# NyanCAD/Cadnip.jl

Hardware: AMD Instinct MI355X
Metric: newton_iters_per_sec (higher is better)
Workload: dtype f64; 1 GPU; gf180 DFF transient 0-700 ns (synthetic sp_mos1 level-1 card, 30 MOSFETs, n=235, nnz=1090), 4096 Vdd x temp corner instances per GPU (state resident in HBM; one 8-instance workgroup per CU in flight, the rest handed out by the kernel's instance queue); step = DC init + full transient of the batch; instances_per_gpu=4096, instances_total=4096, fused=2, newton_mode=1, launches_last_step=5120, accepted_last_step=6078488, rejected_last_step=692364

## Files before the change

### cadnip.jl_amd/csrc/api.hip

```cpp
#include <hip/hip_runtime.h>
#include <functional>
#include <algorithm>
#include <initializer_list>
#include <stdio.h>
#include <string.h>
#include <string>
#include <vector>
#include "internal.hpp"
#include "lu_transpose.hpp"
#include "va_generated.hpp"

using namespace cadnip;

namespace {
template <class T>
int dev_alloc(T** p, size_t count) {
  if (count == 0) count = 1;
  HIP_TRY(hipMalloc((void**)p, count * sizeof(T)));
  HIP_TRY(hipMemset(*p, 0, count * sizeof(T)));
  return CADNIP_OK;
}
template <class T>
int dev_upload(T** p, const T* src, size_t count) {
  int rc = dev_alloc(p, count);
// ... 949 lines not shown
int cadnip_sync(CadnipHandle* h) { if (!h) return CADNIP_BADARG; HIP_TRY(hipStreamSynchronize(h->stream)); return CADNIP_OK; }

int cadnip_profile_enable(CadnipHandle* h, int32_t on) {
  if (!h) return CADNIP_BADARG;
  h->prof_on = on != 0;
  h->prof.clear();
  return CADNIP_OK;
}
int cadnip_profile_read(CadnipHandle* h, int32_t max_entries, const char** names, double* ms, int64_t* calls) {
  if (!h) return 0;
  int k = 0;
  for (auto& e : h->prof) { if (k >= max_entries) break; names[k] = e.name; ms[k] = e.ms; calls[k] = e.calls; ++k; }
  return k;
}

}

namespace cadnip {
int restore_masks(CadnipHandle* h, bool cold) {
  const std::vector<int> ones((size_t)h->B, 1);
  if (cold) HIP_TRY(hipMemcpy(h->d_cold, ones.data(), ones.size() * sizeof(int), hipMemcpyHostToDevice));
  HIP_TRY(hipMemcpy(h->d_active, ones.data(), ones.size() * sizeof(int), hipMemcpyHostToDevice));
  return CADNIP_OK;
}

int upload_homotopy(CadnipHandle* h, const double* gshunt, const double* srcfact) {
  ++h->graph_epoch;
  const size_t B = (size_t)h->B;
  std::vector<double> g(B, h->spec.gshunt), sf(B, h->spec.srcFact);
  if (gshunt) g.assign(gshunt, gshunt + B);
  if (srcfact) sf.assign(srcfact, srcfact + B);
  bool any = false;
  for (size_t i = 0; i < B; ++i) if (g[i] != 0.0 || sf[i] < 1.0) any = true;
  HIP_TRY(hipMemcpy(h->d_gshunt, g.data(), B * sizeof(double), hipMemcpyHostToDevice));
  HIP_TRY(hipMemcpy(h->d_srcfact, sf.data(), B * sizeof(double), hipMemcpyHostToDevice));
  HIP_TRY(hipStreamSynchronize(h->stream));
  h->homotopy = any;
  return CADNIP_OK;
}
int upload_lu(CadnipHandle* h) {
  ++h->graph_epoch;
  LUProgram& P = h->lu;
  int** olds[] = {&h->d_load_src, &h->d_load_dst, &h->d_ent_pos, &h->d_ent_diag, &h->d_ent_ptr, &h->d_term_a, &h->d_term_b, &h->d_lev_ptr,
                  &h->d_lu_rowptr, &h->d_lu_col, &h->d_lu_diag, &h->d_rperm, &h->d_cperm, &h->d_fwd_rows, &h->d_fwd_lev_ptr, &h->d_bwd_rows, &h->d_bwd_lev_ptr};
  for (int** p : olds) if (*p) { (void)hipFree(*p); *p = nullptr; }
  if (h->d_LU) { (void)hipFree(h->d_LU); h->d_LU = nullptr; }
  std::vector<int> dst(h->nnz, 0);
  for (size_t k = 0; k < P.load_src.size(); ++k) dst[P.load_src[k]] = P.load_dst[k];
  TRY(dev_upload(&h->d_load_dst, dst));
  TRY(dev_upload(&h->d_ent_pos, P.ent_pos)); TRY(dev_upload(&h->d_ent_diag, P.ent_diag)); TRY(dev_upload(&h->d_ent_ptr, P.ent_ptr));
  TRY(dev_upload(&h->d_term_a, P.term_a)); TRY(dev_upload(&h->d_term_b, P.term_b)); TRY(dev_upload(&h->d_lev_ptr, P.lev_ptr));
  TRY(dev_upload(&h->d_lu_rowptr, P.lu_rowptr)); TRY(dev_upload(&h->d_lu_col, P.lu_col)); TRY(dev_upload(&h->d_lu_diag, P.lu_diag));
  TRY(dev_upload(&h->d_rperm, P.rperm)); TRY(dev_upload(&h->d_cperm, P.cperm));
  TRY(dev_upload(&h->d_fwd_rows, P.fwd_rows)); TRY(dev_upload(&h->d_fwd_lev_ptr, P.fwd_lev_ptr));
  TRY(dev_upload(&h->d_bwd_rows, P.bwd_rows)); TRY(dev_upload(&h->d_bwd_lev_ptr, P.bwd_lev_ptr));
  TRY(dev_alloc(&h->d_LU, (size_t)h->B * P.nnz_lu));
  h->analyzed = true;
  h->f2.dirty = true;
  h->ac.dirty = true;
  return CADNIP_OK;
}
}
```

### cadnip.jl_amd/csrc/dc_chain.hpp

```cpp
#pragma once
#include <algorithm>
#include <cmath>
#include <cstddef>
#include <vector>

namespace cadnip {

struct DCLogEntry { int inst, stage; double value; int ok; long long iters; };

struct DCChainOpts {
  int use_pcnr, cold_start, fused, use_stepping;
  bool has_limits;
  double gshunt, srcFact;
  const int* participate;
};

struct DCRun {
  int stage, use_pcnr, cold_start, fused;
  const int* part;
  const double* u;
  const double *gshunt, *srcFact;
  int* status;
  long long* iters;
  double *R, *R_direct;
  int B;
  double* dest() const {
    if (!R_direct) return R;
    for (int i = 0; i < B; ++i) if (status[i] != 1) return R;
    return R_direct;
  }
};

struct DCChainResult {
  long long iters = 0;
  int n_failed = 0;
  bool direct = false;
// ... 24 lines not shown
      s.factor = std::sqrt(s.factor);
    }
    return s.steps >= 20 ? GAVE_UP : AGAIN;
  }
};

struct SourceRule {
  struct State { double src = 0.0, conv = 0.0, raise = 0.1; int steps = 0; };
  double value(const State& s) const { return s.src; }
  Next digest(State& s, bool ok) const {
    ++s.steps;
    if (ok) {
      s.conv = s.src;
      if (s.src >= 1.0) return SOLVED;
      s.src = std::fmin(s.src + s.raise, 1.0);
    } else {
      if (s.src - s.conv < 1e-6) return GAVE_UP;
      s.raise /= 2.0;
      s.src = s.conv + s.raise;
    }
    return s.steps >= 50 ? GAVE_UP : AGAIN;
  }
};

template <class Rule> struct Ladder { typename Rule::State s; bool over = false; std::vector<double> u; };

}

template <class Runner>
int dc_chain(const DCChainOpts& o, int B_, int n_, double* u, int* converged, Runner&& runner, std::vector<DCLogEntry>& log, DCChainResult& res) {
  using namespace dc_chain_detail;
  const size_t B = (size_t)B_, n = (size_t)n_;
  res = DCChainResult();
  std::vector<double> start, U, R(B * n);
  std::vector<int> fin(B, 0), status(B), part(B, 1);
  std::vector<long long> iters(B);
  std::vector<double> gsh(B, o.gshunt), sfc(B, o.srcFact);
  auto masked = [&](size_t i) { return o.participate && !o.participate[i]; };
  for (size_t i = 0; i < B; ++i) if (masked(i)) { part[i] = 0; fin[i] = 1; }
  auto n_open = [&]() { int k = 0; for (size_t i = 0; i < B; ++i) k += !fin[i]; return k; };
  auto row = [&](std::vector<double>& v, size_t i) { return v.begin() + i * n; };
  auto run = [&](int stage, int use_pcnr, int cold_start, int fused, const double* from, const double* rung, double* R_direct) -> int {
    const DCRun r{stage, use_pcnr, cold_start, fused, part.data(), from, gsh.data(), sfc.data(), status.data(), iters.data(), R.data(), R_direct, B_};
    if (int rc = runner(r)) return rc;
    res.direct = R_direct && r.dest() == R_direct;
    for (size_t i = 0; i < B; ++i)
      if (part[i]) { res.iters += iters[i]; log.push_back({(int)i, stage, rung ? rung[i] : 0.0, status[i] == 1 ? 1 : 0, iters[i]}); }
    return 0;
  };
  auto take_all = [&]() { for (size_t i = 0; i < B; ++i) if (part[i]) { std::copy(row(R, i), row(R, i + 1), row(U, i)); if (status[i] == 1) fin[i] = 1; } };
  auto stepping = [&](int stage, auto rule, std::vector<double>& term, double spec_value) -> int {
    std::vector<Ladder<decltype(rule)>> L(B);
    for (size_t i = 0; i < B; ++i) { L[i].over = fin[i]; if (!fin[i]) L[i].u.assign(n, 0.0); }
    for (;;) {
      int k = 0;
      for (size_t i = 0; i < B; ++i) {
        part[i] = !L[i].over;
        term[i] = part[i] ? rule.value(L[i].s) : spec_value;
        if (part[i]) { ++k; std::copy(L[i].u.begin(), L[i].u.end(), row(U, i)); }
      }
      if (!k) return 0;
      if (int rc = run(stage, 0, 0, 0, U.data(), term.data(), nullptr)) return rc;
      for (size_t i = 0; i < B; ++i) {
        if (!part[i]) continue;
        const bool ok = status[i] == 1;
        if (ok) L[i].u.assign(row(R, i), row(R, i + 1));
        const Next next = rule.digest(L[i].s, ok);
        if (next == AGAIN) continue;
        L[i].over = true;
        fin[i] = next == SOLVED;
        std::copy(L[i].u.begin(), L[i].u.end(), row(U, i));
      }
    }
  };
  if (n_open())
    if (int rc = run(0, o.use_pcnr, o.cold_start, o.fused, u, nullptr, o.participate ? nullptr : u)) return rc;
  if (res.direct) {
    if (converged) std::fill(converged, converged + B, 1);
    return 0;
  }
  start.assign(u, u + B * n);
  U = start;
  take_all();
  if (n_open() && o.use_pcnr && o.has_limits) {
    for (size_t i = 0; i < B; ++i) { part[i] = !fin[i]; if (part[i]) std::copy(row(start, i), row(start, i + 1), row(U, i)); }
    if (int rc = run(1, 0, 0, 0, U.data(), nullptr, nullptr)) return rc;
    take_all();
  }
  if (n_open() && o.use_stepping)
    if (int rc = stepping(2, GshuntRule(o.gshunt), gsh, o.gshunt)) return rc;
  if (n_open() && o.use_stepping)
    if (int rc = stepping(3, SourceRule(), sfc, o.srcFact)) return rc;
  res.n_failed = n_open();
  std::copy(U.begin(), U.end(), u);
  if (converged) for (size_t i = 0; i < B; ++i) converged[i] = masked(i) ? 0 : fin[i];
  return 0;
}

}
```

### cadnip.jl_amd/csrc/driver.hip

```cpp
#include <hip/hip_runtime.h>
#include <chrono>
#include <string.h>
#include <vector>
#include "internal.hpp"
#include "dc_chain.hpp"

using namespace cadnip;

struct Driver {
  int n_save = 0, n_obs = 0, n_break = 0;
  double *t = nullptr, *h = nullptr, *hprev = nullptr, *hpp = nullptr;
  int *nhist = nullptr, *order = nullptr, *k = nullptr, *status = nullptr, *bp_idx = nullptr, *save_idx = nullptr, *dcstate = nullptr, *action = nullptr;
  long long* cnt = nullptr;
  double *mn_a0f = nullptr, *mn_ss = nullptr, *mn_dnp = nullptr; int* mn_flags = nullptr;
  double *u0 = nullptr, *u1 = nullptr, *u2 = nullptr, *up = nullptr, *beta = nullptr;
  double *u3 = nullptr, *hp3 = nullptr;
  double *atol = nullptr, *emask = nullptr, *breaks = nullptr, *save_t = nullptr, *out = nullptr;
  int* obs = nullptr;
  int* nactive = nullptr;
  int* part = nullptr;
  size_t out_cap = 0, brk_cap = 0, save_cap = 0, obs_cap = 0;
  std::vector<DCLogEntry> dc_log;
};

namespace {
#define TRY(x) do { int _rc = (x); if (_rc) return _rc; } while (0)
template <class T> int dalloc(T** p, size_t c) { if (*p) return CADNIP_OK; HIP_TRY(hipMalloc((void**)p, (c ? c : 1) * sizeof(T))); HIP_TRY(hipMemset(*p, 0, (c ? c : 1) * sizeof(T))); return CADNIP_OK; }
template <class T> int drealloc(T** p, size_t* cap, size_t c) { if (*p && *cap >= c) return CADNIP_OK; if (*p) (void)hipFree(*p); *p = nullptr; *cap = c; return dalloc(p, c); }

template <class F> int each_buffer(Driver* d, size_t B, size_t n, F f) {
  const size_t later = 0;
  TRY(f(&d->t, B)); TRY(f(&d->h, B)); TRY(f(&d->hprev, B)); TRY(f(&d->hpp, B));
  TRY(f(&d->nhist, B)); TRY(f(&d->order, B)); TRY(f(&d->k, B)); TRY(f(&d->status, B));
  TRY(f(&d->bp_idx, B)); TRY(f(&d->save_idx, B)); TRY(f(&d->dcstate, B)); TRY(f(&d->action, B));
  TRY(f(&d->cnt, B * 4));
  TRY(f(&d->mn_a0f, B)); TRY(f(&d->mn_ss, B)); TRY(f(&d->mn_dnp, B)); TRY(f(&d->mn_flags, B));
  TRY(f(&d->u0, B * n)); TRY(f(&d->u1, B * n)); TRY(f(&d->u2, B * n)); TRY(f(&d->up, B * n)); TRY(f(&d->beta, B * n));
  TRY(f(&d->atol, n)); TRY(f(&d->emask, n)); TRY(f(&d->nactive, 2)); TRY(f(&d->part, B));
  TRY(f(&d->u3, later)); TRY(f(&d->hp3, later));
  TRY(f(&d->breaks, later)); TRY(f(&d->save_t, later)); TRY(f(&d->obs, later)); TRY(f(&d->out, later));
  return CADNIP_OK;
}

int ensure_driver(CadnipHandle* h) {
  if (!h->drv) h->drv = new Driver();
  return each_buffer(h->drv, h->B, h->n, [](auto** p, size_t c) { return c ? dalloc(p, c) : CADNIP_OK; });
}

}
#include "tran_ctrl.hpp"
namespace {
__global__ void __launch_bounds__(64) k_tran_init(TranArgs a) {
  const int inst = blockIdx.x, tid = threadIdx.x, n = a.n;
  double* u = a.u + (size_t)inst * n;
  double* u0 = a.u0 + (size_t)inst * n;
  for (int i = tid; i < n; i += 64) { double v = u[i]; u0[i] = v; a.u1[(size_t)inst * n + i] = v; a.u2[(size_t)inst * n + i] = v; }
  int bp = 0;
  while (bp < a.n_break && a.breaks[bp] <= a.t0) ++bp;
  int si = 0;
  while (si < a.n_save && a.save_t[si] <= a.t0) {
    double* o = a.out + ((size_t)inst * a.n_save + si) * a.n_obs;
// ... 205 lines not shown
      for (int i = 0; i < h->B && victim < 0; ++i) if (stat[i] == -2) victim = i;
      if (victim >= 0) {
        ++repivots;
        std::vector<int> act((size_t)h->B);
        for (int i = 0; i < h->B; ++i) act[i] = (stat[i] == 0 || stat[i] == -2) ? 1 : 0;
        HIP_TRY(hipMemcpy(h->d_active, act.data(), act.size() * sizeof(int), hipMemcpyHostToDevice));
        rc = launch_jacobian(h); if (rc) break;
        HIP_TRY(hipStreamSynchronize(h->stream));
        if (cadnip_analyze(h, victim) == CADNIP_OK) {
          for (int i = 0; i < h->B; ++i) if (stat[i] == -2) stat[i] = 0;
          HIP_TRY(hipMemcpy(d->status, stat.data(), stat.size() * sizeof(int), hipMemcpyHostToDevice));
          rc = count_running(h, &running); if (rc) break;
        } else {
          for (int i = 0; i < h->B; ++i) act[i] = stat[i] == 0 ? 1 : 0;
          HIP_TRY(hipMemcpy(h->d_active, act.data(), act.size() * sizeof(int), hipMemcpyHostToDevice));
        }
      }
    }
    prev_running = running;
    if (running == 0) break;
  }
  h->initjct = saved_initjct;
  return rc;
}

}

extern "C" {

void cadnip_driver_free(CadnipHandle* h) {
  if (!h || !h->drv) return;
  Driver* d = h->drv;
  (void)each_buffer(d, 0, 0, [](auto** p, size_t) { if (*p) (void)hipFree(*p); return CADNIP_OK; });
  delete d;
  h->drv = nullptr;
}

int cadnip_tran_state(CadnipHandle* h, double* t_host, double* h_host, int32_t* order_host) {
  if (!h || !h->drv) return CADNIP_NOTREADY;
  Driver* d = h->drv;
  size_t B = h->B;
  if (t_host) HIP_TRY(hipMemcpy(t_host, d->t, B * sizeof(double), hipMemcpyDeviceToHost));
  if (h_host) HIP_TRY(hipMemcpy(h_host, d->h, B * sizeof(double), hipMemcpyDeviceToHost));
  if (order_host) HIP_TRY(hipMemcpy(order_host, d->order, B * sizeof(int), hipMemcpyDeviceToHost));
  return CADNIP_OK;
}

int cadnip_dc_run(CadnipHandle* h, const CadnipDCOpts* o, double* u_host, int32_t* converged_host, CadnipRunStats* st) {
  if (!h || !o || !u_host) return CADNIP_BADARG;
  TRY(ensure_driver(h));
  Driver* d = h->drv;
  const size_t B = h->B, n = h->n;
  auto w0 = std::chrono::steady_clock::now();
  d->dc_log.clear();
  if (!h->analyzed) {
    HIP_TRY(hipMemcpy(h->d_u, u_host, B * n * sizeof(double), hipMemcpyHostToDevice));
    TRY(restore_masks(h, false));
    TRY_RC(dev_zero_async(h, h->d_gamma, B * sizeof(double)));
    TRY_RC(dev_zero_async(h, h->d_t, B * sizeof(double)));
    std::vector<double> g(B, 1e9);
    int ij = h->initjct;
    h->initjct = (o->cold_start && o->use_pcnr && h->n_limits > 0) ? 1 : 0;
    int rc = launch_rebuild(h);
    h->initjct = ij;
    if (rc) return rc;
    HIP_TRY(hipMemcpy(h->d_gamma, g.data(), B * sizeof(double), hipMemcpyHostToDevice));
    TRY(launch_jacobian(h));
    HIP_TRY(hipStreamSynchronize(h->stream));
    TRY(cadnip_analyze(h, 0));
  }
  struct HomotopyGuard {
    CadnipHandle* h;
    ~HomotopyGuard() { (void)upload_homotopy(h, nullptr, nullptr); }
  } guard{h};
  std::vector<long long> cnt(B * 4);
  auto device_run = [&](const DCRun& r) -> int {
    HIP_TRY(hipMemcpy(h->d_u, r.u, B * n * sizeof(double), hipMemcpyHostToDevice));
    HIP_TRY(hipMemcpy(d->part, r.part, B * sizeof(int), hipMemcpyHostToDevice));
    TRY(upload_homotopy(h, r.gshunt, r.srcFact));
    TRY(dc_newton(h, o->abstol, o->maxiters, r.use_pcnr, r.cold_start, r.fused, d->part));
    HIP_TRY(hipMemcpy(r.status, d->status, B * sizeof(int), hipMemcpyDeviceToHost));
    HIP_TRY(hipMemcpy(r.dest(), h->d_u, B * n * sizeof(double), hipMemcpyDeviceToHost));
    HIP_TRY(hipMemcpy(cnt.data(), d->cnt, B * 4 * sizeof(long long), hipMemcpyDeviceToHost));
    for (size_t i = 0; i < B; ++i) r.iters[i] = cnt[i * 4];
    return CADNIP_OK;
  };
  const DCChainOpts chain{o->use_pcnr, o->cold_start, o->fused, o->use_stepping, h->n_limits > 0, h->spec.gshunt, h->spec.srcFact, o->participate};
  DCChainResult res;
  TRY(dc_chain(chain, h->B, h->n, u_host, converged_host, device_run, d->dc_log, res));
  if (!res.direct) HIP_TRY(hipMemcpy(h->d_u, u_host, B * n * sizeof(double), hipMemcpyHostToDevice));
  TRY(restore_masks(h, true));
  if (st) {
    memset(st, 0, sizeof(*st));
    st->newton_iters = res.iters;
    st->n_failed = res.n_failed;
    st->wall_seconds = std::chrono::duration<double>(std::chrono::steady_clock::now() - w0).count();
  }
  return res.n_failed ? CADNIP_NOCONV : CADNIP_OK;
}

int32_t cadnip_dc_log_size(CadnipHandle* h) { return (h && h->drv) ? (int32_t)h->drv->dc_log.size() : 0; }
int cadnip_dc_log_get(CadnipHandle* h, int32_t* inst, int32_t* stage, double* value, int32_t* ok, int64_t* iters) {
  if (!h || !h->drv) return CADNIP_NOTREADY;
  size_t k = 0;
  for (auto& e : h->drv->dc_log) {
    if (inst) inst[k] = e.inst; if (stage) stage[k] = e.stage; if (value) value[k] = e.value; if (ok) ok[k] = e.ok; if (iters) iters[k] = e.iters;
    ++k;
  }
  return CADNIP_OK;
}

int cadnip_tran_run(CadnipHandle* h, const CadnipTranOpts* o, double* out_host, int64_t* per_inst_host, CadnipRunStats* st) {
  if (!h || !o || !o->abstol || o->t1 <= o->t0 || o->n_save < 0 || o->n_break < 0) return CADNIP_BADARG;
  if (!h->analyzed) return CADNIP_NOTREADY;
  for (int i = 1; i < o->n_break; ++i) if (!(o->breaks[i] > o->breaks[i - 1])) return CADNIP_BADARG;
  for (int i = 1; i < o->n_save; ++i) if (!(o->save_t[i] >= o->save_t[i - 1])) return CADNIP_BADARG;
  for (int i = 0; i < o->n_obs; ++i) if (o->obs[i] < 0 || o->obs[i] >= h->n) return CADNIP_BADARG;
  TRY(ensure_driver(h));
  Driver* d = h->drv;
  const size_t B = h->B, n = h->n;
  const int n_obs = o->n_obs > 0 ? o->n_obs : (int)n;
  TRY(drealloc(&d->breaks, &d->brk_cap, (size_t)o->n_break));
  TRY(drealloc(&d->save_t, &d->save_cap, (size_t)o->n_save));
  TRY(drealloc(&d->obs, &d->obs_cap, (size_t)n_obs));
  TRY(drealloc(&d->out, &d->out_cap, B * (size_t)o->n_save * n_obs));
  if (o->n_break) HIP_TRY(hipMemcpy(d->breaks, o->breaks, o->n_break * sizeof(double), hipMemcpyHostToDevice));
  if (o->n_save) HIP_TRY(hipMemcpy(d->save_t, o->save_t, o->n_save * sizeof(double), hipMemcpyHostToDevice));
  std::vector<int> obs(n_obs);
  for (int i = 0; i < n_obs; ++i) obs[i] = o->n_obs > 0 ? o->obs[i] : i;
  HIP_TRY(hipMemcpy(d->obs, obs.data(), n_obs * sizeof(int), hipMemcpyHostToDevice));
  HIP_TRY(hipMemcpy(d->atol, o->abstol, n * sizeof(double), hipMemcpyHostToDevice));
  std::vector<double> emask(n, 1.0);
  int n_err = (int)n;
  if (o->err_mask) { n_err = 0; for (size_t i = 0; i < n; ++i) { emask[i] = o->err_mask[i] != 0.0 ? 1.0 : 0.0; n_err += emask[i] != 0.0; } }
  HIP_TRY(hipMemcpy(d->emask, emask.data(), n * sizeof(double), hipMemcpyHostToDevice));
  HIP_TRY(hipStreamSynchronize(h->stream));
  if (o->max_order >= 3) { TRY(dalloc(&d->u3, B * n)); TRY(dalloc(&d->hp3, B)); }
  TranArgs a = tran_args(h, o, n_obs, n_err);
  const bool delayed = h->dly.n_term > 0;
  if (delayed) { a.hmax = fmin(a.hmax, h->dly.tau_min); a.h0 = fmin(a.h0, a.hmax); }
  struct DelayGuard { CadnipHandle* h; bool on; ~DelayGuard() { if (on) { (void)launch_delay_clear(h); (void)hipStreamSynchronize(h->stream); } } } delay_guard{h, delayed};
  const bool use_fused = o->fused && fused2_plan(h, F2_TRAN, o->newton_mode).circuit_ok;
  struct ModeGuard { CadnipHandle* h; int saved; ~ModeGuard() { h->spec.mode = saved; } } mode_guard{h, h->spec.mode};
  h->spec.mode = 1;
  hipLaunchKernelGGL(k_tran_init, dim3(h->B), dim3(64), 0, h->stream, a);
  if (delayed) TRY(launch_delay_init(h, a.t0));
  HIP_TRY(hipStreamSynchronize(h->stream));
  auto w0 = std::chrono::steady_clock::now();
  int64_t launches = 0;
  const int64_t max_it = o->max_iterations > 0 ? o->max_iterations : 50000000;
  int rc = CADNIP_OK, running = h->B;
  const int check_every = use_fused ? 1024 : 8;
  if (use_fused) {
    hipEvent_t ev[2] = {nullptr, nullptr};
    HIP_TRY(hipEventCreateWithFlags(&ev[0], hipEventDisableTiming));
    HIP_TRY(hipEventCreateWithFlags(&ev[1], hipEventDisableTiming));
    int slot = 0;
    bool have_prev = false;
    while (launches < max_it) {
      rc = launch_fused2_rounds(h, a, check_every); if (rc) break;
      launches += check_every;
      rc = enqueue_running_count(h, slot); if (rc) break;
      if (hipEventRecord(ev[slot], h->stream) != hipSuccess) { rc = CADNIP_HIPERROR; break; }
      if (have_prev) {
        if (hipEventSynchronize(ev[1 - slot]) != hipSuccess) { rc = CADNIP_HIPERROR; break; }
        running = ((volatile int*)h->h_pinned)[1 - slot];
        if (running == 0) break;
      }
      have_prev = true;
      slot ^= 1;
    }
    hipError_t es = hipStreamSynchronize(h->stream);
    (void)hipEventDestroy(ev[0]); (void)hipEventDestroy(ev[1]);
    if (es != hipSuccess) { set_last_error("hipStreamSynchronize", es); return CADNIP_HIPERROR; }
    if (!rc && running > 0) rc = count_running(h, &running);
  }
  while (!use_fused && running > 0 && launches < max_it) {
    for (int c = 0; c < check_every; ++c) {
      rc = launch_rebuild(h); if (rc) break;
      if (delayed) { rc = launch_delay_apply(h, d->status); if (rc) break; }
      rc = launch_residual(h, h->d_du); if (rc) break;
      rc = launch_factor_solve(h, true, h->d_resid, h->d_delta); if (rc) break;
      { ProfScope ps(h, "tran_update");
        if (h->n >= 4096) hipLaunchKernelGGL(k_tran_update<256>, dim3(h->B), dim3(256), 0, h->stream, a);
        else hipLaunchKernelGGL(k_tran_update<64>, dim3(h->B), dim3(64), 0, h->stream, a); }
      if (delayed) { rc = launch_delay_record(h, d->t, d->u0, d->status); if (rc) break; }
      ++launches;
    }
    if (rc) break;
    rc = count_running(h, &running); if (rc) break;
  }
  HIP_TRY(hipStreamSynchronize(h->stream));
  double wall = std::chrono::duration<double>(std::chrono::steady_clock::now() - w0).count();
  if (rc) return rc;
  std::vector<long long> cnt(B * 4);
  std::vector<int> status(B);
  HIP_TRY(hipMemcpy(cnt.data(), d->cnt, B * 4 * sizeof(long long), hipMemcpyDeviceToHost));
  HIP_TRY(hipMemcpy(status.data(), d->status, B * sizeof(int), hipMemcpyDeviceToHost));
  if (out_host && o->n_save) HIP_TRY(hipMemcpy(out_host, d->out, B * (size_t)o->n_save * n_obs * sizeof(double), hipMemcpyDeviceToHost));
  CadnipRunStats s; memset(&s, 0, sizeof(s));
  for (size_t i = 0; i < B; ++i) {
    s.newton_iters += cnt[i * 4 + 0]; s.steps_accepted += cnt[i * 4 + 1]; s.steps_rejected += cnt[i * 4 + 2]; s.newton_failures += cnt[i * 4 + 3];
    if (status[i] != 1) s.n_failed += 1;
    if (per_inst_host) { per_inst_host[i * 4 + 0] = cnt[i * 4 + 0]; per_inst_host[i * 4 + 1] = cnt[i * 4 + 1]; per_inst_host[i * 4 + 2] = cnt[i * 4 + 2]; per_inst_host[i * 4 + 3] = status[i]; }
  }
  s.launches = launches; s.wall_seconds = wall;
  if (st) *st = s;
  TRY(restore_masks(h, false));
  return s.n_failed ? CADNIP_NOCONV : CADNIP_OK;
}

}
```

### cadnip.jl_amd/csrc/internal.hpp

```cpp
#pragma once
#include <hip/hip_runtime.h>
#include <stdint.h>
#include <string>
#include <vector>
#include "../../include/cadnip_hip.h"
#include "stamp_plan.hpp"
#include "ac_hbm_plan.hpp"
#include "delay_plan.hpp"
#define CADNIP_MOS1_PAR_OXCAP 8
#define CADNIP_MOS1_PAR_GD 30
#define CADNIP_MOS1_PAR_GS 31

#define HIP_TRY(expr)                                                     \
  do {                                                                    \
    hipError_t _e = (expr);                                               \
    if (_e != hipSuccess) {                                               \
      cadnip::set_last_error(#expr, _e);                                  \
      return CADNIP_HIPERROR;                                             \
    }                                                                     \
  } while (0)

namespace cadnip {

void set_last_error(const char* what, hipError_t e);
// ... 130 lines not shown
  template <class F> void each_buffer(F f) {
    f((void**)&d_pos); f((void**)&d_taps); f((void**)&d_rows); f((void**)&d_row_ptr); f((void**)&d_term_tap); f((void**)&d_row_store);
    f((void**)&d_tau); f((void**)&d_w); f((void**)&d_W); f((void**)&d_hist_t); f((void**)&d_hist_v); f((void**)&d_v_init);
    f((void**)&d_head); f((void**)&d_count);
  }
};

}

struct CadnipHandle {
  int device = 0;
  hipStream_t stream = nullptr;
  int B = 0;
  int n = 0, n_nodes = 0, n_currents = 0, n_charges = 0, n_limits = 0, nnz = 0;
  std::vector<int> h_rowptr, h_colidx, h_to_ref;
  std::vector<int> h_g_ptr, h_g_slots, h_c_ptr, h_c_slots, h_b_ptr, h_b_slots;
  int ns_g = 0, ns_c = 0, ns_b = 0, ns = 0;
  std::vector<cadnip::DeviceBlock> blocks;
  std::vector<double> h_limit_init;
  CadnipSpec spec{1, 1e-12, 0.0, 1.0};
  int initjct = 0;
  int *d_rowptr = nullptr, *d_colidx = nullptr, *d_to_ref = nullptr;
  int *d_g_ptr = nullptr, *d_g_slots = nullptr, *d_c_ptr = nullptr, *d_c_slots = nullptr, *d_b_ptr = nullptr, *d_b_slots = nullptr;
  unsigned char* d_diag_flag = nullptr;
  int* d_long_rows = nullptr;
  int n_long_rows = 0;
  double* d_dump = nullptr;
  unsigned* d_prep = nullptr;
  int n_prep = 0, n_prep_atomic = 0;
  bool prep_stale = true;
  double* d_wave = nullptr;
  double* d_limit_init = nullptr;
  double *d_gshunt = nullptr, *d_srcfact = nullptr;
  bool homotopy = false;
  double *d_u = nullptr, *d_du = nullptr, *d_t = nullptr, *d_gamma = nullptr;
  double *d_G = nullptr, *d_C = nullptr, *d_b = nullptr, *d_J = nullptr, *d_resid = nullptr, *d_delta = nullptr;
  double *d_limit_w = nullptr, *d_LU = nullptr, *d_tmp = nullptr;
  int* d_flags = nullptr;
  int* d_active = nullptr;
  int* d_nonfinite = nullptr;
  int* d_cold = nullptr;
  bool analyzed = false;
  cadnip::LUProgram lu;
  int *d_load_src = nullptr, *d_load_dst = nullptr, *d_ent_pos = nullptr, *d_ent_diag = nullptr, *d_ent_ptr = nullptr;
  int *d_term_a = nullptr, *d_term_b = nullptr, *d_lev_ptr = nullptr;
  int *d_lu_rowptr = nullptr, *d_lu_col = nullptr, *d_lu_diag = nullptr, *d_rperm = nullptr, *d_cperm = nullptr;
  int *d_fwd_rows = nullptr, *d_fwd_lev_ptr = nullptr, *d_bwd_rows = nullptr, *d_bwd_lev_ptr = nullptr;
  std::vector<unsigned char> leaf_unit_ok;
  cadnip::LULeaves leaves;
  bool va_ext = false;
  cadnip::FusedState f2;
  cadnip::AcState ac;
  cadnip::DelayState dly;
  struct Driver* drv = nullptr;
  bool prof_on = false;
  std::vector<cadnip::ProfEntry> prof;
  hipEvent_t ev0 = nullptr, ev1 = nullptr;
  int* h_pinned = nullptr;
  int* d_pinned = nullptr;
  char* h_stage = nullptr; char* d_stage = nullptr; size_t stage_bytes = 0, stage_off = 0;
  struct PendingDown { void* dst; const void* src; size_t bytes; };
  struct StepGraph { hipGraphExec_t exec = nullptr; unsigned long long epoch = 0, warmed = 0; };
  StepGraph step_graph[4];
  unsigned long long graph_epoch = 1;
  std::vector<PendingDown> stage_pending;
};
// ... 76 lines not shown
```

### cadnip.jl_amd/hip.py

```python
import ctypes as C
import os

import numpy as np

from .structure import Structure, TYPE_ID, type_id

_HERE = os.path.dirname(os.path.abspath(__file__))
LIB_PATH = os.environ.get("CADNIP_HIP_LIB") or os.path.join(_HERE, "libcadnip_hip.so")

OK, BADARG, SINGULAR, NONFINITE, HIPERROR, NOTREADY, NOCONV = range(7)
STATUS_NAMES = {0: "CADNIP_OK", 1: "CADNIP_BADARG", 2: "CADNIP_SINGULAR", 3: "CADNIP_NONFINITE",
                4: "CADNIP_HIPERROR", 5: "CADNIP_NOTREADY", 6: "CADNIP_NOCONV"}

AC_BREAKDOWN_TOL = 6e-9
AC_MEMORY = {"lds": 0, "hbm": 1, "auto": 2}

EXPORTS = [
    "cadnip_create", "cadnip_destroy", "cadnip_set_params", "cadnip_set_spec", "cadnip_set_initjct",
    "cadnip_rebuild", "cadnip_residual", "cadnip_jacobian", "cadnip_jacobian_dense", "cadnip_ode_rhs", "cadnip_ode_jacobian", "cadnip_get_GCb", "cadnip_get_contributions", "cadnip_analyze",
    "cadnip_analyze_values", "cadnip_factor", "cadnip_solve", "cadnip_factor_solve", "cadnip_lu_order", "cadnip_ac_solve", "cadnip_ac_adjoint", "cadnip_ac_solve_multi", "cadnip_ac_adjoint_multi", "cadnip_ac_sens", "cadnip_ac_arnoldi", "cadnip_ac_set_memory", "cadnip_ac_set_overlay", "cadnip_ac_plan_info", "cadnip_newton_step", "cadnip_newton_step_fused", "cadnip_debug_step_time", "cadnip_lu_stats", "cadnip_dc_run",
    "cadnip_dc_log_size", "cadnip_dc_log_get", "cadnip_tran_set_delay", "cadnip_tran_delay_info", "cadnip_tran_run", "cadnip_tran_state", "cadnip_dev_ptr", "cadnip_stream", "cadnip_set_u", "cadnip_get_u", "cadnip_get_flags",
    "cadnip_sync", "cadnip_debug_copy", "cadnip_debug_stamp_time", "cadnip_profile_enable", "cadnip_profile_read", "cadnip_version",
    "cadnip_host_lu_analyze", "cadnip_host_lu_analyze_leaves", "cadnip_host_lu_size", "cadnip_host_lu_blocks", "cadnip_host_lu_get", "cadnip_host_lu_free", "cadnip_host_lu_transpose",
    "cadnip_host_f2_build", "cadnip_host_f2_size", "cadnip_host_f2_get", "cadnip_host_f2_free", "cadnip_host_f2_team_steps", "cadnip_host_f2_steps",
# ... 5 lines not shown
        self.code = code
        super().__init__("%s returned %s" % (where, STATUS_NAMES.get(code, code)))


class SingularException(CadnipError):
    """Maps CADNIP_SINGULAR like the Julia shim maps it to LinearAlgebra.SingularException."""


class DeviceBlockC(C.Structure):
    _fields_ = [("type", C.c_int32), ("count", C.c_int32),
                ("n_nodes", C.c_int32), ("nodes", C.POINTER(C.c_int32)),
                ("n_ipar", C.c_int32), ("ipar", C.POINTER(C.c_int32)),
                ("n_par", C.c_int32),
                ("g_base", C.c_int32), ("c_base", C.c_int32), ("b_base", C.c_int32),
                ("n_g", C.c_int32), ("n_c", C.c_int32), ("n_b", C.c_int32)]


_I = C.POINTER(C.c_int32)
_D = C.POINTER(C.c_double)


class StructureC(C.Structure):
    _fields_ = [("n", C.c_int32), ("n_nodes", C.c_int32), ("n_currents", C.c_int32), ("n_charges", C.c_int32),
                ("n_limits", C.c_int32), ("nnz", C.c_int32), ("rowptr", _I), ("colidx", _I), ("to_ref_nz", _I),
                ("n_blocks", C.c_int32), ("blocks", C.POINTER(DeviceBlockC)),
                ("n_wave_data", C.c_int32), ("wave_data", _D),
                ("ns_g", C.c_int32), ("ns_c", C.c_int32), ("ns_b", C.c_int32),
                ("g_ptr", _I), ("g_slots", _I), ("c_ptr", _I), ("c_slots", _I), ("b_ptr", _I), ("b_slots", _I),
                ("diag_nz", _I), ("limit_init", _D)]


class SpecC(C.Structure):
    _fields_ = [("mode", C.c_int32), ("gmin", C.c_double), ("gshunt", C.c_double), ("srcFact", C.c_double)]


class DCOptsC(C.Structure):
    _fields_ = [("abstol", C.c_double), ("maxiters", C.c_int32), ("use_pcnr", C.c_int32), ("cold_start", C.c_int32),
                ("use_stepping", C.c_int32), ("fused", C.c_int32), ("participate", _I)]


class TranOptsC(C.Structure):
    _fields_ = [("t0", C.c_double), ("t1", C.c_double), ("reltol", C.c_double), ("abstol", _D), ("err_mask", _D), ("h0", C.c_double),
                ("hmin", C.c_double), ("hmax", C.c_double), ("max_newton", C.c_int32), ("max_order", C.c_int32),
                ("use_pcnr", C.c_int32), ("newton_tol", C.c_double), ("n_break", C.c_int32), ("breaks", _D),
                ("n_save", C.c_int32), ("save_t", _D), ("n_obs", C.c_int32), ("obs", _I),
                ("max_iterations", C.c_int64), ("fused", C.c_int32), ("newton_mode", C.c_int32), ("step_rule", C.c_int32)]


class DelaySpecC(C.Structure):
    _fields_ = [("n_pos", C.c_int32), ("pos", _I), ("n_term", C.c_int32), ("term_pos", _I), ("term_row", _I), ("term_col", _I),
                ("tau", _D), ("w", _D), ("depth", C.c_int32)]


TRAN_DELAY_OVERFLOW = -4


class RunStatsC(C.Structure):
    _fields_ = [("newton_iters", C.c_int64), ("steps_accepted", C.c_int64), ("steps_rejected", C.c_int64),
                ("newton_failures", C.c_int64), ("launches", C.c_int64), ("n_failed", C.c_int32),
                ("wall_seconds", C.c_double)]


_lib = None


def _share_hip_runtime():
# ... 349 lines not shown
                                          _dp(berr), _ip(flags), _ip(info)), "cadnip_ac_arnoldi")
        return H, beta, meff, ll, V, berr, flags, _ac_info(info)

    def ac_set_memory(self, mode="lds", max_waves=0):
        code = AC_MEMORY.get(mode, -1) if isinstance(mode, str) else int(mode)
        _check(self.lib.cadnip_ac_set_memory(self.h, C.c_int32(code), C.c_int32(int(max_waves))), "cadnip_ac_set_memory")

    def ac_set_overlay(self, pos, omegas, val):
        ps = np.ascontiguousarray(np.asarray(pos, dtype=np.int32).ravel())
        om = np.ascontiguousarray(np.asarray(omegas, dtype=np.float64).ravel())
        if ps.size == 0:
            return self.ac_clear_overlay()
        vv = np.asarray(val, dtype=np.complex128)
        if vv.shape not in ((om.size, ps.size), (self.B, om.size, ps.size)):
            raise ValueError("val must be [F, O] or [B, F, O] for F frequencies and O positions")
        vv = np.ascontiguousarray(np.broadcast_to(vv, (self.B, om.size, ps.size)))
        _check(self.lib.cadnip_ac_set_overlay(self.h, C.c_int32(ps.size), _ip(ps), C.c_int32(om.size), _dp(om), vv.ctypes.data_as(_D)), "cadnip_ac_set_overlay")

    def ac_clear_overlay(self):
        _check(self.lib.cadnip_ac_set_overlay(self.h, C.c_int32(0), None, C.c_int32(0), None, None), "cadnip_ac_set_overlay")

    def ac_plan_info(self):
        out = (C.c_int64 * 4)()
        _check(self.lib.cadnip_ac_plan_info(self.h, out), "cadnip_ac_plan_info")
        return dict(memory={v: k for k, v in AC_MEMORY.items()}[int(out[0])], n_waves=int(out[1]), work_bytes=int(out[2]), lds_bytes=int(out[3]))

    def lu_stats(self):
        v = [C.c_int32() for _ in range(5)]
        _check(self.lib.cadnip_lu_stats(self.h, *[C.byref(x) for x in v]), "cadnip_lu_stats")
        return dict(zip(("nnz_lu", "n_terms", "n_levels", "n_fwd_levels", "n_bwd_levels"), [x.value for x in v]))

    def dc_run(self, u0=None, abstol=1e-10, maxiters=100, use_pcnr=True, cold_start=True, use_stepping=True,
               raise_on_fail=False, fused=False, participate=None):
        u = self._bn(0.0 if u0 is None else u0).copy()
        conv = np.zeros(self.B, dtype=np.int32)
        st = RunStatsC()
        pm = None if participate is None else np.ascontiguousarray(np.asarray(participate, dtype=bool).astype(np.int32))
        o = DCOptsC(abstol, maxiters, int(use_pcnr), int(cold_start), int(use_stepping), int(fused), None if pm is None else _ip(pm))
        rc = self.lib.cadnip_dc_run(self.h, C.byref(o), _dp(u), _ip(conv), C.byref(st))
        if rc not in (OK, NOCONV) or (rc == NOCONV and raise_on_fail):
            _check(rc, "cadnip_dc_run")
        return u, conv.astype(bool), _stats(st)

    def dc_log(self):
        k = int(self.lib.cadnip_dc_log_size(self.h))
        inst, stage, ok = (np.zeros(max(k, 1), dtype=np.int32) for _ in range(3))
        val, it = np.zeros(max(k, 1)), np.zeros(max(k, 1), dtype=np.int64)
        _check(self.lib.cadnip_dc_log_get(self.h, _ip(inst), _ip(stage), _dp(val), _ip(ok), it.ctypes.data_as(C.POINTER(C.c_int64))), "cadnip_dc_log_get")
        return [(int(inst[j]), int(stage[j]), float(val[j]), bool(ok[j]), int(it[j])) for j in range(k)]

    def tran_run(self, t0, t1, abstol, reltol=1e-4, breaks=(), save_t=(), obs=None, h0=0.0, hmin=0.0, hmax=0.0,
                 max_newton=10, max_order=2, use_pcnr=False, newton_tol=1e-3, max_iterations=0, fused=False,
                 err_mask="differential", newton_mode=0, step_rule=0):
        at = np.ascontiguousarray(np.broadcast_to(np.asarray(abstol, dtype=np.float64), (self.st.n,)))
        if isinstance(err_mask, str):
            em = self.st.differential_mask() if err_mask == "differential" else np.ones(self.st.n)
        else:
            em = np.ones(self.st.n) if err_mask is None else np.asarray(err_mask, dtype=np.float64)
        em = np.ascontiguousarray(em, dtype=np.float64)
        br = np.ascontiguousarray(np.asarray(breaks, dtype=np.float64))
        sv = np.ascontiguousarray(np.asarray(save_t, dtype=np.float64))
        ob = np.ascontiguousarray(np.asarray(obs if obs is not None else [], dtype=np.int32))
        n_obs = ob.size if ob.size else self.st.n
        out = np.zeros((self.B, sv.size, n_obs))
        per = np.zeros((self.B, 4), dtype=np.int64)
        st = RunStatsC()
        o = TranOptsC(t0, t1, reltol, _dp(at), _dp(em), h0, hmin, hmax, max_newton, max_order, int(use_pcnr), newton_tol,
                      br.size, _dp(br) if br.size else None, sv.size, _dp(sv) if sv.size else None,
                      ob.size, _ip(ob) if ob.size else None, max_iterations, int(fused), int(newton_mode), int(step_rule))
        rc = self.lib.cadnip_tran_run(self.h, C.byref(o), _dp(out), per.ctypes.data_as(C.POINTER(C.c_int64)), C.byref(st))
        if rc not in (OK, NOCONV):
# ... 150 lines not shown
```

### include/cadnip_hip.h

```cpp
#ifndef CADNIP_HIP_H
#define CADNIP_HIP_H

#include <stdint.h>

#ifdef __cplusplus
extern "C" {
#endif

typedef enum {
  CADNIP_OK = 0,
  CADNIP_BADARG = 1,
  CADNIP_SINGULAR = 2,
  CADNIP_NONFINITE = 3,
  CADNIP_HIPERROR = 4,
  CADNIP_NOTREADY = 5,
  CADNIP_NOCONV = 6
} CadnipStatus;

typedef enum {
  CADNIP_DEV_RESISTOR = 0,
  CADNIP_DEV_CAPACITOR = 1,
  CADNIP_DEV_INDUCTOR = 2,
  CADNIP_DEV_VSOURCE = 3,
  CADNIP_DEV_ISOURCE = 4,
// ... 103 lines not shown
                    int32_t* info );
int cadnip_ac_adjoint(CadnipHandle* h, int32_t n_freq, const double* omega , double gmin, const double* c_host ,
                      int32_t n_pairs, const int32_t* pairs , int32_t wpb, double* h_host ,
                      double* x_host , double* berr_host , int32_t* flags_host ,
                      int32_t* info );
int cadnip_ac_solve_multi(CadnipHandle* h, int32_t n_freq, const double* omega , double gmin, int32_t n_rhs,
                          const double* b_host , int32_t n_pairs, const int32_t* pairs ,
                          int32_t wpb, double* h_host , double* x_host ,
                          double* berr_host , int32_t* flags_host , int32_t* info );
int cadnip_ac_adjoint_multi(CadnipHandle* h, int32_t n_freq, const double* omega , double gmin, int32_t n_rhs,
                            const double* c_host , int32_t n_pairs, const int32_t* pairs ,
                            int32_t wpb, double* h_host , double* x_host ,
                            double* berr_host , int32_t* flags_host , int32_t* info );
int cadnip_ac_sens(CadnipHandle* h, int32_t n_freq, const double* omega , double gmin, int32_t n_base, const int32_t* base ,
                   int32_t n_par, const int32_t* plus , const int32_t* minus , const double* scale ,
                   const double* bac_host , const double* db_host , const double* c_host ,
                   const int32_t* pair , int32_t wpb, double* y_host , double* s_host ,
                   double* x_host , double* berr_host ,
                   int32_t* flags_host , int32_t* info );
int cadnip_ac_arnoldi(CadnipHandle* h, int32_t n_shift, const double* omega , double gmin, const double* b_host , int32_t m,
                      double breakdown_tol, int32_t n_pairs, const int32_t* pairs , int32_t wpb,
                      double* H_host , double* beta_host , int32_t* meff_host ,
                      double* l_host , double* v_host ,
                      double* berr_host , int32_t* flags_host , int32_t* info );

#define CADNIP_AC_LDS 0
#define CADNIP_AC_HBM 1
#define CADNIP_AC_AUTO 2
int cadnip_ac_set_memory(CadnipHandle* h, int32_t mode, int32_t max_waves);
int cadnip_ac_set_overlay(CadnipHandle* h, int32_t n_ovl, const int32_t* pos , int32_t n_freq, const double* omega ,
                          const double* val );
int cadnip_ac_plan_info(CadnipHandle* h, int64_t out[4]);

typedef struct {
  double abstol;
  int32_t maxiters;
  int32_t use_pcnr;
  int32_t cold_start;
  int32_t use_stepping;
  int32_t fused;
  const int32_t* participate;
} CadnipDCOpts;

typedef struct {
  double t0, t1;
  double reltol;
  const double* abstol;
  const double* err_mask;
  double h0;
  double hmin, hmax;
  int32_t max_newton;
  int32_t max_order;
  int32_t use_pcnr;
  double newton_tol;
  int32_t n_break; const double* breaks;
  int32_t n_save;  const double* save_t;
  int32_t n_obs;   const int32_t* obs;
  int64_t max_iterations;
  int32_t fused;
  int32_t newton_mode;
  int32_t step_rule;
} CadnipTranOpts;

typedef struct {
  int64_t newton_iters;
  int64_t steps_accepted, steps_rejected, newton_failures;
// ... 69 lines not shown
```

Baseline: 183.7 million newton_iters/s.

## Cache uploaded options, stage transfers through pinned memory, zero-start DC on device

```diff
diff --git a/cadnip.jl_amd/csrc/api.hip b/cadnip.jl_amd/csrc/api.hip
--- a/cadnip.jl_amd/csrc/api.hip
+++ b/cadnip.jl_amd/csrc/api.hip
@@ -1005,9 +1005,18 @@
   if (srcfact) sf.assign(srcfact, srcfact + B);
   bool any = false;
   for (size_t i = 0; i < B; ++i) if (g[i] != 0.0 || sf[i] < 1.0) any = true;
-  HIP_TRY(hipMemcpy(h->d_gshunt, g.data(), B * sizeof(double), hipMemcpyHostToDevice));
-  HIP_TRY(hipMemcpy(h->d_srcfact, sf.data(), B * sizeof(double), hipMemcpyHostToDevice));
-  HIP_TRY(hipStreamSynchronize(h->stream));
+  bool sent = false;
+  auto put = [&](double* dev, std::vector<double>& held, const std::vector<double>& v) -> int {
+    if (held.size() == B && memcmp(held.data(), v.data(), B * sizeof(double)) == 0) return CADNIP_OK;
+    held.clear();
+    HIP_TRY(hipMemcpy(dev, v.data(), B * sizeof(double), hipMemcpyHostToDevice));
+    held = v;
+    sent = true;
+    return CADNIP_OK;
+  };
+  TRY_RC(put(h->d_gshunt, h->held_gshunt, g));
+  TRY_RC(put(h->d_srcfact, h->held_srcfact, sf));
+  if (sent) HIP_TRY(hipStreamSynchronize(h->stream));
   h->homotopy = any;
   return CADNIP_OK;
 }
diff --git a/cadnip.jl_amd/csrc/dc_chain.hpp b/cadnip.jl_amd/csrc/dc_chain.hpp
--- a/cadnip.jl_amd/csrc/dc_chain.hpp
+++ b/cadnip.jl_amd/csrc/dc_chain.hpp
@@ -2,6 +2,8 @@
 #include <algorithm>
 #include <cmath>
 #include <cstddef>
+#include <limits>
+#include <memory>
 #include <vector>
 
 namespace cadnip {
@@ -92,7 +94,14 @@
   using namespace dc_chain_detail;
   const size_t B = (size_t)B_, n = (size_t)n_;
   res = DCChainResult();
-  std::vector<double> start, U, R(B * n);
+  std::vector<double> start, U;
+  const std::unique_ptr<double[]> R_store(new double[B * n]);
+  double* const R = R_store.get();
+#ifdef CADNIP_DC_CHAIN_POISON
+  std::fill(R, R + B * n, std::numeric_limits<double>::quiet_NaN());
+#endif
+  const bool zero_start = o.cold_start == 2 && !o.participate;
+  const int cold_start = o.cold_start == 2 && !zero_start ? 1 : o.cold_start;
   std::vector<int> fin(B, 0), status(B), part(B, 1);
   std::vector<long long> iters(B);
   std::vector<double> gsh(B, o.gshunt), sfc(B, o.srcFact);
@@ -100,15 +109,16 @@
   for (size_t i = 0; i < B; ++i) if (masked(i)) { part[i] = 0; fin[i] = 1; }
   auto n_open = [&]() { int k = 0; for (size_t i = 0; i < B; ++i) k += !fin[i]; return k; };
   auto row = [&](std::vector<double>& v, size_t i) { return v.begin() + i * n; };
+  auto Rrow = [&](size_t i) { return R + i * n; };
   auto run = [&](int stage, int use_pcnr, int cold_start, int fused, const double* from, const double* rung, double* R_direct) -> int {
-    const DCRun r{stage, use_pcnr, cold_start, fused, part.data(), from, gsh.data(), sfc.data(), status.data(), iters.data(), R.data(), R_direct, B_};
+    const DCRun r{stage, use_pcnr, cold_start, fused, part.data(), from, gsh.data(), sfc.data(), status.data(), iters.data(), R, R_direct, B_};
     if (int rc = runner(r)) return rc;
     res.direct = R_direct && r.dest() == R_direct;
     for (size_t i = 0; i < B; ++i)
       if (part[i]) { res.iters += iters[i]; log.push_back({(int)i, stage, rung ? rung[i] : 0.0, status[i] == 1 ? 1 : 0, iters[i]}); }
     return 0;
   };
-  auto take_all = [&]() { for (size_t i = 0; i < B; ++i) if (part[i]) { std::copy(row(R, i), row(R, i + 1), row(U, i)); if (status[i] == 1) fin[i] = 1; } };
+  auto take_all = [&]() { for (size_t i = 0; i < B; ++i) if (part[i]) { std::copy(Rrow(i), Rrow(i + 1), row(U, i)); if (status[i] == 1) fin[i] = 1; } };
   auto stepping = [&](int stage, auto rule, std::vector<double>& term, double spec_value) -> int {
     std::vector<Ladder<decltype(rule)>> L(B);
     for (size_t i = 0; i < B; ++i) { L[i].over = fin[i]; if (!fin[i]) L[i].u.assign(n, 0.0); }
@@ -124,7 +134,7 @@
       for (size_t i = 0; i < B; ++i) {
         if (!part[i]) continue;
         const bool ok = status[i] == 1;
-        if (ok) L[i].u.assign(row(R, i), row(R, i + 1));
+        if (ok) L[i].u.assign(Rrow(i), Rrow(i + 1));
         const Next next = rule.digest(L[i].s, ok);
         if (next == AGAIN) continue;
         L[i].over = true;
@@ -134,12 +144,13 @@
     }
   };
   if (n_open())
-    if (int rc = run(0, o.use_pcnr, o.cold_start, o.fused, u, nullptr, o.participate ? nullptr : u)) return rc;
+    if (int rc = run(0, o.use_pcnr, cold_start, o.fused, zero_start ? nullptr : u, nullptr, o.participate ? nullptr : u)) return rc;
   if (res.direct) {
     if (converged) std::fill(converged, converged + B, 1);
     return 0;
   }
-  start.assign(u, u + B * n);
+  if (zero_start) start.assign(B * n, 0.0);
+  else start.assign(u, u + B * n);
   U = start;
   take_all();
   if (n_open() && o.use_pcnr && o.has_limits) {
diff --git a/cadnip.jl_amd/csrc/driver.hip b/cadnip.jl_amd/csrc/driver.hip
--- a/cadnip.jl_amd/csrc/driver.hip
+++ b/cadnip.jl_amd/csrc/driver.hip
@@ -21,12 +21,46 @@
   int* part = nullptr;
   size_t out_cap = 0, brk_cap = 0, save_cap = 0, obs_cap = 0;
   std::vector<DCLogEntry> dc_log;
+  template <class T> struct Held { std::vector<T> v; bool is = false; };
+  Held<double> held_breaks, held_save_t, held_atol, held_emask;
+  Held<int> held_obs;
+  hipEvent_t ev[2] = {nullptr, nullptr};
+  void* stage = nullptr; size_t stage_cap = 0;
 };
 
 namespace {
 #define TRY(x) do { int _rc = (x); if (_rc) return _rc; } while (0)
 template <class T> int dalloc(T** p, size_t c) { if (*p) return CADNIP_OK; HIP_TRY(hipMalloc((void**)p, (c ? c : 1) * sizeof(T))); HIP_TRY(hipMemset(*p, 0, (c ? c : 1) * sizeof(T))); return CADNIP_OK; }
-template <class T> int drealloc(T** p, size_t* cap, size_t c) { if (*p && *cap >= c) return CADNIP_OK; if (*p) (void)hipFree(*p); *p = nullptr; *cap = c; return dalloc(p, c); }
+template <class T> int drealloc(T** p, size_t* cap, size_t c, bool* held = nullptr) { if (*p && *cap >= c) return CADNIP_OK; if (held) *held = false; if (*p) (void)hipFree(*p); *p = nullptr; *cap = c; return dalloc(p, c); }
+template <class T> int sync_option(T* dev, Driver::Held<T>& held, const T* src, size_t c, bool* sent) {
+  if (held.is && held.v.size() == c && (c == 0 || memcmp(held.v.data(), src, c * sizeof(T)) == 0)) return CADNIP_OK;
+  held.is = false;
+  if (c) { HIP_TRY(hipMemcpy(dev, src, c * sizeof(T), hipMemcpyHostToDevice)); *sent = true; }
+  held.v.assign(src, src + c);
+  held.is = true;
+  return CADNIP_OK;
+}
+
+int stage_fit(Driver* d, size_t bytes) {
+  if (d->stage && d->stage_cap >= bytes) return CADNIP_OK;
+  if (d->stage) (void)hipHostFree(d->stage);
+  d->stage = nullptr; d->stage_cap = 0;
+  HIP_TRY(hipHostMalloc(&d->stage, bytes ? bytes : 1, hipHostMallocDefault));
+  d->stage_cap = bytes ? bytes : 1;
+  return CADNIP_OK;
+}
+int to_caller(CadnipHandle* h, void* dst, const void* dev, size_t bytes) {
+  TRY(stage_fit(h->drv, bytes));
+  HIP_TRY(hipMemcpy(h->drv->stage, dev, bytes, hipMemcpyDeviceToHost));
+  memcpy(dst, h->drv->stage, bytes);
+  return CADNIP_OK;
+}
+int from_caller(CadnipHandle* h, void* dev, const void* src, size_t bytes) {
+  TRY(stage_fit(h->drv, bytes));
+  memcpy(h->drv->stage, src, bytes);
+  HIP_TRY(hipMemcpy(dev, h->drv->stage, bytes, hipMemcpyHostToDevice));
+  return CADNIP_OK;
+}
 
 template <class F> int each_buffer(Driver* d, size_t B, size_t n, F f) {
   const size_t later = 0;
@@ -298,6 +332,8 @@
   if (!h || !h->drv) return;
   Driver* d = h->drv;
   (void)each_buffer(d, 0, 0, [](auto** p, size_t) { if (*p) (void)hipFree(*p); return CADNIP_OK; });
+  for (hipEvent_t e : d->ev) if (e) (void)hipEventDestroy(e);
+  if (d->stage) (void)hipHostFree(d->stage);
   delete d;
   h->drv = nullptr;
 }
@@ -319,8 +355,10 @@
   const size_t B = h->B, n = h->n;
   auto w0 = std::chrono::steady_clock::now();
   d->dc_log.clear();
+  const bool zero_start = o->cold_start == CADNIP_DC_COLD_ZERO && !o->participate;
   if (!h->analyzed) {
-    HIP_TRY(hipMemcpy(h->d_u, u_host, B * n * sizeof(double), hipMemcpyHostToDevice));
+    if (zero_start) TRY_RC(dev_zero_async(h, h->d_u, B * n * sizeof(double)));
+    else TRY(from_caller(h, h->d_u, u_host, B * n * sizeof(double)));
     TRY(restore_masks(h, false));
     TRY_RC(dev_zero_async(h, h->d_gamma, B * sizeof(double)));
     TRY_RC(dev_zero_async(h, h->d_t, B * sizeof(double)));
@@ -341,20 +379,21 @@
   } guard{h};
   std::vector<long long> cnt(B * 4);
   auto device_run = [&](const DCRun& r) -> int {
-    HIP_TRY(hipMemcpy(h->d_u, r.u, B * n * sizeof(double), hipMemcpyHostToDevice));
+    if (r.u) TRY(from_caller(h, h->d_u, r.u, B * n * sizeof(double)));
+    else TRY_RC(dev_zero_async(h, h->d_u, B * n * sizeof(double)));
     HIP_TRY(hipMemcpy(d->part, r.part, B * sizeof(int), hipMemcpyHostToDevice));
     TRY(upload_homotopy(h, r.gshunt, r.srcFact));
     TRY(dc_newton(h, o->abstol, o->maxiters, r.use_pcnr, r.cold_start, r.fused, d->part));
-    HIP_TRY(hipMemcpy(r.status, d->status, B * sizeof(int), hipMemcpyDeviceToHost));
-    HIP_TRY(hipMemcpy(r.dest(), h->d_u, B * n * sizeof(double), hipMemcpyDeviceToHost));
-    HIP_TRY(hipMemcpy(cnt.data(), d->cnt, B * 4 * sizeof(long long), hipMemcpyDeviceToHost));
+    TRY(to_caller(h, r.status, d->status, B * sizeof(int)));
+    TRY(to_caller(h, r.dest(), h->d_u, B * n * sizeof(double)));
+    TRY(to_caller(h, cnt.data(), d->cnt, B * 4 * sizeof(long long)));
     for (size_t i = 0; i < B; ++i) r.iters[i] = cnt[i * 4];
     return CADNIP_OK;
   };
   const DCChainOpts chain{o->use_pcnr, o->cold_start, o->fused, o->use_stepping, h->n_limits > 0, h->spec.gshunt, h->spec.srcFact, o->participate};
   DCChainResult res;
   TRY(dc_chain(chain, h->B, h->n, u_host, converged_host, device_run, d->dc_log, res));
-  if (!res.direct) HIP_TRY(hipMemcpy(h->d_u, u_host, B * n * sizeof(double), hipMemcpyHostToDevice));
+  if (!res.direct) TRY(from_caller(h, h->d_u, u_host, B * n * sizeof(double)));
   TRY(restore_masks(h, true));
   if (st) {
     memset(st, 0, sizeof(*st));
@@ -386,21 +425,22 @@
   Driver* d = h->drv;
   const size_t B = h->B, n = h->n;
   const int n_obs = o->n_obs > 0 ? o->n_obs : (int)n;
-  TRY(drealloc(&d->breaks, &d->brk_cap, (size_t)o->n_break));
-  TRY(drealloc(&d->save_t, &d->save_cap, (size_t)o->n_save));
-  TRY(drealloc(&d->obs, &d->obs_cap, (size_t)n_obs));
+  TRY(drealloc(&d->breaks, &d->brk_cap, (size_t)o->n_break, &d->held_breaks.is));
+  TRY(drealloc(&d->save_t, &d->save_cap, (size_t)o->n_save, &d->held_save_t.is));
+  TRY(drealloc(&d->obs, &d->obs_cap, (size_t)n_obs, &d->held_obs.is));
   TRY(drealloc(&d->out, &d->out_cap, B * (size_t)o->n_save * n_obs));
-  if (o->n_break) HIP_TRY(hipMemcpy(d->breaks, o->breaks, o->n_break * sizeof(double), hipMemcpyHostToDevice));
-  if (o->n_save) HIP_TRY(hipMemcpy(d->save_t, o->save_t, o->n_save * sizeof(double), hipMemcpyHostToDevice));
+  bool sent = false;
+  TRY(sync_option(d->breaks, d->held_breaks, o->breaks, (size_t)o->n_break, &sent));
+  TRY(sync_option(d->save_t, d->held_save_t, o->save_t, (size_t)o->n_save, &sent));
   std::vector<int> obs(n_obs);
   for (int i = 0; i < n_obs; ++i) obs[i] = o->n_obs > 0 ? o->obs[i] : i;
-  HIP_TRY(hipMemcpy(d->obs, obs.data(), n_obs * sizeof(int), hipMemcpyHostToDevice));
-  HIP_TRY(hipMemcpy(d->atol, o->abstol, n * sizeof(double), hipMemcpyHostToDevice));
+  TRY(sync_option(d->obs, d->held_obs, (const int*)obs.data(), (size_t)n_obs, &sent));
+  TRY(sync_option(d->atol, d->held_atol, o->abstol, n, &sent));
   std::vector<double> emask(n, 1.0);
   int n_err = (int)n;
   if (o->err_mask) { n_err = 0; for (size_t i = 0; i < n; ++i) { emask[i] = o->err_mask[i] != 0.0 ? 1.0 : 0.0; n_err += emask[i] != 0.0; } }
-  HIP_TRY(hipMemcpy(d->emask, emask.data(), n * sizeof(double), hipMemcpyHostToDevice));
-  HIP_TRY(hipStreamSynchronize(h->stream));
+  TRY(sync_option(d->emask, d->held_emask, (const double*)emask.data(), n, &sent));
+  if (sent) HIP_TRY(hipStreamSynchronize(h->stream));
   if (o->max_order >= 3) { TRY(dalloc(&d->u3, B * n)); TRY(dalloc(&d->hp3, B)); }
   TranArgs a = tran_args(h, o, n_obs, n_err);
   const bool delayed = h->dly.n_term > 0;
@@ -418,9 +458,8 @@
   int rc = CADNIP_OK, running = h->B;
   const int check_every = use_fused ? 1024 : 8;
   if (use_fused) {
-    hipEvent_t ev[2] = {nullptr, nullptr};
-    HIP_TRY(hipEventCreateWithFlags(&ev[0], hipEventDisableTiming));
-    HIP_TRY(hipEventCreateWithFlags(&ev[1], hipEventDisableTiming));
+    hipEvent_t* const ev = d->ev;
+    for (int s = 0; s < 2; ++s) if (!ev[s]) HIP_TRY(hipEventCreateWithFlags(&ev[s], hipEventDisableTiming));
     int slot = 0;
     bool have_prev = false;
     while (launches < max_it) {
@@ -437,7 +476,6 @@
       slot ^= 1;
     }
     hipError_t es = hipStreamSynchronize(h->stream);
-    (void)hipEventDestroy(ev[0]); (void)hipEventDestroy(ev[1]);
     if (es != hipSuccess) { set_last_error("hipStreamSynchronize", es); return CADNIP_HIPERROR; }
     if (!rc && running > 0) rc = count_running(h, &running);
   }
@@ -461,9 +499,9 @@
   if (rc) return rc;
   std::vector<long long> cnt(B * 4);
   std::vector<int> status(B);
-  HIP_TRY(hipMemcpy(cnt.data(), d->cnt, B * 4 * sizeof(long long), hipMemcpyDeviceToHost));
-  HIP_TRY(hipMemcpy(status.data(), d->status, B * sizeof(int), hipMemcpyDeviceToHost));
-  if (out_host && o->n_save) HIP_TRY(hipMemcpy(out_host, d->out, B * (size_t)o->n_save * n_obs * sizeof(double), hipMemcpyDeviceToHost));
+  TRY(to_caller(h, cnt.data(), d->cnt, B * 4 * sizeof(long long)));
+  TRY(to_caller(h, status.data(), d->status, B * sizeof(int)));
+  if (out_host && o->n_save) TRY(to_caller(h, out_host, d->out, B * (size_t)o->n_save * n_obs * sizeof(double)));
   CadnipRunStats s; memset(&s, 0, sizeof(s));
   for (size_t i = 0; i < B; ++i) {
     s.newton_iters += cnt[i * 4 + 0]; s.steps_accepted += cnt[i * 4 + 1]; s.steps_rejected += cnt[i * 4 + 2]; s.newton_failures += cnt[i * 4 + 3];
diff --git a/cadnip.jl_amd/csrc/internal.hpp b/cadnip.jl_amd/csrc/internal.hpp
--- a/cadnip.jl_amd/csrc/internal.hpp
+++ b/cadnip.jl_amd/csrc/internal.hpp
@@ -186,6 +186,7 @@
   double* d_wave = nullptr;
   double* d_limit_init = nullptr;
   double *d_gshunt = nullptr, *d_srcfact = nullptr;
+  std::vector<double> held_gshunt, held_srcfact;
   bool homotopy = false;
   double *d_u = nullptr, *d_du = nullptr, *d_t = nullptr, *d_gamma = nullptr;
   double *d_G = nullptr, *d_C = nullptr, *d_b = nullptr, *d_J = nullptr, *d_resid = nullptr, *d_delta = nullptr;
diff --git a/cadnip.jl_amd/hip.py b/cadnip.jl_amd/hip.py
--- a/cadnip.jl_amd/hip.py
+++ b/cadnip.jl_amd/hip.py
@@ -61,6 +61,9 @@
 
 class SpecC(C.Structure):
     _fields_ = [("mode", C.c_int32), ("gmin", C.c_double), ("gshunt", C.c_double), ("srcFact", C.c_double)]
+
+
+DC_COLD_ZERO = 2
 
 
 class DCOptsC(C.Structure):
@@ -476,11 +479,12 @@
 
     def dc_run(self, u0=None, abstol=1e-10, maxiters=100, use_pcnr=True, cold_start=True, use_stepping=True,
                raise_on_fail=False, fused=False, participate=None):
-        u = self._bn(0.0 if u0 is None else u0).copy()
+        zero = u0 is None and bool(cold_start) and participate is None
+        u = np.empty((self.B, self.st.n)) if zero else self._bn(0.0 if u0 is None else u0).copy()
         conv = np.zeros(self.B, dtype=np.int32)
         st = RunStatsC()
         pm = None if participate is None else np.ascontiguousarray(np.asarray(participate, dtype=bool).astype(np.int32))
-        o = DCOptsC(abstol, maxiters, int(use_pcnr), int(cold_start), int(use_stepping), int(fused), None if pm is None else _ip(pm))
+        o = DCOptsC(abstol, maxiters, int(use_pcnr), DC_COLD_ZERO if zero else int(cold_start), int(use_stepping), int(fused), None if pm is None else _ip(pm))
         rc = self.lib.cadnip_dc_run(self.h, C.byref(o), _dp(u), _ip(conv), C.byref(st))
         if rc not in (OK, NOCONV) or (rc == NOCONV and raise_on_fail):
             _check(rc, "cadnip_dc_run")
diff --git a/include/cadnip_hip.h b/include/cadnip_hip.h
--- a/include/cadnip_hip.h
+++ b/include/cadnip_hip.h
@@ -159,6 +159,7 @@
                           const double* val );
 int cadnip_ac_plan_info(CadnipHandle* h, int64_t out[4]);
 
+#define CADNIP_DC_COLD_ZERO 2
 typedef struct {
   double abstol;
   int32_t maxiters;
```

Measured after the change: 188.3 million newton_iters/s, median of 6. 1.02x the previous value.
